# ateme-developers/SVT-AV1-1

Hardware: AMD Instinct MI355X
Metric: 64x64 SAD-search blocks/sec (higher is better)
Workload: dtype u8; 1 GPU; configs[1]: 64x64 full-pel SAD hierarchical ME (centre check + HME L0/L1/L2 + 64x64-area full-pel search of 85 square PUs), 1080p 8-bit, one reference list

## Files before the change

### svt-av1-1_amd/csrc/me_hme.hip

```cpp
#include <hip/hip_runtime.h>
#include <stdint.h>

#include "../../include/svtav1_hip.h"
#include "me_kernels.h"

namespace svthip {

namespace {
#include "me_hme_impl.h"
}

__global__ void __launch_bounds__(256) hme_center_kernel(const uint8_t* __restrict__ pool, HmeJobTable jobs, svthip_me_params P,
                                                         uint32_t list_index, const svthip_sb_origin* __restrict__ sbs, uint32_t n_sb,
                                                         uint32_t n_jobs, const uint32_t* __restrict__ l0_best_mv64, uint32_t l0_mv_stride,
                                                         svthip_fullpel_desc* __restrict__ out_desc,
                                                         int16_t* __restrict__ out_center, int16_t* __restrict__ hme_state)
{
    __shared__ HmeShared sh;
    __shared__ __attribute__((aligned(16))) uint8_t hme_lds[4 * kHmeLdsPerWave];
    const uint32_t sbi = xcd_item(blockIdx.x, n_sb * n_jobs);
    if (sbi >= n_sb * n_jobs) return;
    const uint32_t job = sbi / n_sb, sb_local = sbi - job * n_sb;
    hme_center_sb(pool, jobs.cur[job], jobs.ref[job], P, list_index, sbs[sb_local].x, sbs[sb_local].y, sbi, l0_best_mv64,
                  l0_mv_stride, out_desc, out_center, hme_state, sh, hme_lds);
}

#ifdef SVTHIP_HME_STAMPS
extern "C" int svthip_debug_hme_stamps(void* host, size_t bytes)
{
    return (int)hipMemcpyFromSymbol(host, HIP_SYMBOL(g_hme_stamps), bytes < sizeof(g_hme_stamps) ? bytes : sizeof(g_hme_stamps));
}
extern "C" int svthip_debug_hme_loop_phases(unsigned long long* host8)
{
    return (int)hipMemcpyFromSymbol(host8, HIP_SYMBOL(g_hme_loop_phase), sizeof(g_hme_loop_phase));
}
#endif

}
```

### svt-av1-1_amd/csrc/me_hme_impl.h

```cpp
#pragma once


typedef const __attribute__((address_space(1))) uint32_t gmem_u32;
struct __attribute__((packed, aligned(1))) gmem_u32x4 { uint32_t v[4]; };

__device__ __forceinline__ uint32_t ldu32(const uint8_t* p)
{
    const uintptr_t a = reinterpret_cast<uintptr_t>(p);
    gmem_u32* q = (gmem_u32*)(a & ~(uintptr_t)3);
    const uint32_t sh = (uint32_t)(a & 3u);
    const uint32_t lo = q[0];
    const uint32_t hi = sh ? q[1] : 0u;
    return __builtin_amdgcn_alignbyte(hi, lo, sh);
}

__device__ __forceinline__ uint32_t ldu32_nb(const uint8_t* p)
{
    const uintptr_t a = reinterpret_cast<uintptr_t>(p);
    gmem_u32* q = (gmem_u32*)(a & ~(uintptr_t)3);
    return __builtin_amdgcn_alignbyte(q[1], q[0], (uint32_t)(a & 3u));
}

__device__ __forceinline__ uint32_t wave_sum_u32(uint32_t v)
{
#pragma unroll
    for (int m = 1; m < 64; m <<= 1) v += __shfl_xor(v, m);
    return v;
}

#ifdef SVTHIP_HME_NO_PRIO
#define HME_PRIO(p) do { } while (0)
#else
#define HME_PRIO(p) __builtin_amdgcn_s_setprio(p)
#endif
#ifdef SVTHIP_HME_STAMPS
__device__ unsigned long long g_hme_stamps[8192 * 4 * 8];
#define HME_STAMP(i)                                                                                                          \
    do {                                                                                                                      \
        if (lane == 0 && sbi < 8192u) g_hme_stamps[((size_t)sbi * 4 + (threadIdx.x >> 6)) * 8 + (i)] = __builtin_amdgcn_s_memtime(); \
    } while (0)
__device__ unsigned long long g_hme_loop_phase[2 * 4];
#define HME_LOOP_T(var) const unsigned long long var = __builtin_amdgcn_s_memtime()
#define HME_LOOP_ADD(slot, t1, t0)                                                                                \
    do {                                                                                                          \
        if (lane == 0) atomicAdd(&g_hme_loop_phase[(W == 64 ? 4 : 0) + (slot)], (unsigned long long)((t1) - (t0))); \
    } while (0)
#else
#define HME_STAMP(i) do { } while (0)
#define HME_LOOP_T(var) do { } while (0)
#define HME_LOOP_ADD(slot, t1, t0) do { } while (0)
#endif

__device__ __forceinline__ unsigned long long wave_min_u64(unsigned long long v)
{
#pragma unroll
    for (int m = 1; m < 64; m <<= 1) {
        unsigned long long o = __shfl_xor(v, m);
        v = o < v ? o : v;
    }
    return v;
}

__device__ uint32_t wave_block_sad(const uint8_t* src, uint32_t src_stride, const uint8_t* ref, uint32_t ref_stride,
                                   uint32_t H, uint32_t W, int lane, const uint32_t* src_lds = nullptr)
{
    if (src_lds && W == 64 && H == 32) {
        const uint32_t c = (uint32_t)lane & 15u, r0 = (uint32_t)lane >> 4;
        const uint8_t* rp = ref + (size_t)r0 * ref_stride + 4u * c;
        uint32_t tv[8], acc4 = 0;
#pragma unroll
        for (int k = 0; k < 8; k++) tv[k] = ldu32_nb(rp + (size_t)(4 * k) * ref_stride);
#pragma unroll
        for (int k = 0; k < 8; k++) acc4 = __builtin_amdgcn_sad_u8(src_lds[(r0 + 4 * k) * 16 + c], tv[k], acc4);
        return wave_sum_u32(acc4);
    }
    if (W == 64 && (H & 3u) == 0) {
        const uint32_t c = (uint32_t)lane & 15u, r0 = (uint32_t)lane >> 4;
        const uint8_t* sp = src + (size_t)r0 * src_stride + 4u * c;
        const uint8_t* rp = ref + (size_t)r0 * ref_stride + 4u * c;
        uint32_t acc4 = 0;
        for (uint32_t r = 0; r < H; r += 16) {
            uint32_t sv[4], tv[4];
#pragma unroll
            for (int k = 0; k < 4; k++) {
                const bool in = r + 4u * (uint32_t)k < H;
                sv[k] = in ? *reinterpret_cast<const uint32_t*>(sp + (size_t)(4 * k) * src_stride) : 0u;
                tv[k] = in ? ldu32_nb(rp + (size_t)(4 * k) * ref_stride) : 0u;
            }
#pragma unroll
            for (int k = 0; k < 4; k++) acc4 = __builtin_amdgcn_sad_u8(sv[k], tv[k], acc4);
            sp += (size_t)16 * src_stride;
            rp += (size_t)16 * ref_stride;
        }
        return wave_sum_u32(acc4);
    }
    const uint32_t ndw = (W + 3) >> 2;
    const uint32_t n = H * ndw;
    uint32_t acc = 0;
    for (uint32_t i = lane; i < n; i += 64) {
        const uint32_t r = i / ndw, c = i - r * ndw;
        uint32_t s = ldu32(src + (size_t)r * src_stride + 4 * c);
        uint32_t t = ldu32(ref + (size_t)r * ref_stride + 4 * c);
        const uint32_t rem = W - 4 * c;
        if (rem < 4) {
            const uint32_t m = (1u << (8 * rem)) - 1u;
            s &= m;
            t &= m;
        }
        acc = __builtin_amdgcn_sad_u8(s, t, acc);
    }
    return wave_sum_u32(acc);
}

__device__ void wave_sad_loop_generic(const uint8_t* src, uint32_t src_stride, const uint8_t* ref, uint32_t ref_stride,
                                      uint32_t H, uint32_t W, uint32_t ref_stride_raw, int sw, int sh, int lane,
                                      uint32_t* best_sad, int* bx, int* by)
{
    const int npos = sw * sh;
    unsigned long long best = ~0ull;
    const uint32_t ndw = (W + 3) >> 2;
    const uint32_t tail = W & 3u;
    const uint32_t tailmask = tail ? ((1u << (8 * tail)) - 1u) : 0xffffffffu;
#pragma unroll 1
    for (int pos = lane; pos < npos; pos += 64) {
        const int y = pos / sw, x = pos - y * sw;
        const uint8_t* r0 = ref + (size_t)y * ref_stride_raw + x;
        uint32_t acc = 0;
#pragma unroll 1
        for (uint32_t r = 0; r < H; r++) {
            const uint8_t* sp = src + (size_t)r * src_stride;
            const uint8_t* rp = r0 + (size_t)r * ref_stride;
#pragma unroll 2
            for (uint32_t c = 0; c < ndw; c++) {
                uint32_t s = ldu32(sp + 4 * c);
                uint32_t t = ldu32(rp + 4 * c);
                if (c == ndw - 1) {
                    s &= tailmask;
                    t &= tailmask;
                }
                acc = __builtin_amdgcn_sad_u8(s, t, acc);
            }
        }
        const unsigned long long key = ((unsigned long long)acc << 32) | (uint32_t)pos;
        best = key < best ? key : best;
    }
    best = wave_min_u64(best);
    const uint32_t pos = (uint32_t)__builtin_amdgcn_readfirstlane((int)(uint32_t)best);
    *best_sad = (uint32_t)__builtin_amdgcn_readfirstlane((int)(uint32_t)(best >> 32));
    *by = (int)(pos / (uint32_t)sw);
    *bx = (int)(pos - (uint32_t)(*by) * (uint32_t)sw);
}

__device__ __forceinline__ uint32_t min3u(uint32_t a, uint32_t b, uint32_t c)
{
    uint32_t r;
    asm("v_min3_u32 %0, %1, %2, %3" : "=v"(r) : "v"(a), "v"(b), "v"(c));
    return r;
}

__device__ __forceinline__ uint64_t pack64(uint32_t lo, uint32_t hi) { return ((uint64_t)hi << 32) | lo; }

__device__ __forceinline__ void stage_window_rows(const uint8_t* base, uint32_t ref_stride_raw, int wrows, int pitch, uint32_t* win,
                                                  int lane)
{
    constexpr int NP = 6;
    const int lpr = (pitch + 3) >> 2;
    const int rpp = lpr < 64 ? 64 / lpr : 1;
    const int g = (int)(((uint32_t)lane * ((1u << 16) / (uint32_t)lpr + 1u)) >> 16), q4 = 4 * (lane - g * lpr);
    const bool lane_ok = g < rpp;
    const uintptr_t a0 = reinterpret_cast<uintptr_t>(base) + 4u * (uint32_t)q4;
    for (int r0 = g; r0 < wrows; r0 += NP * rpp) {
        gmem_u32x4 w[NP];
#pragma unroll
        for (int u = 0; u < NP; u++) {
            const int r = min(r0 + u * rpp, wrows - 1);
            const __attribute__((address_space(1))) gmem_u32x4* q = (const __attribute__((address_space(1))) gmem_u32x4*)(a0 + (size_t)r * ref_stride_raw);
#pragma unroll
            for (int k = 0; k < 4; k++) w[u].v[k] = q->v[k];
        }
#pragma unroll
        for (int u = 0; u < NP; u++) {
            const int r = r0 + u * rpp;
            if (lane_ok && r < wrows) {
                uint32_t* o = win + r * pitch + q4;
#pragma unroll
                for (int k = 0; k < 4; k++)
                    if (q4 + k < pitch) o[k] = w[u].v[k];
            }
        }
    }
}

template <int W, bool KEY32 = false>
__device__ void wave_sad_loop_lds(const uint8_t* src, uint32_t src_stride, const uint8_t* ref, uint32_t ref_stride_raw,
                                  int H, int sw, int sh, int lane, uint8_t* lds, int lds_bytes, uint32_t* best_sad,
                                  int* bx, int* by, const uint32_t* shared_src = nullptr)
{
    constexpr int WD = W / 4;
    constexpr int FLUSH = (W == 16) ? 16 : (W == 32 ? 8 : 4);
    const int own_src = shared_src ? 0 : H * WD;
    const uint32_t* srcbuf = shared_src ? shared_src : reinterpret_cast<const uint32_t*>(lds);
    const int noct = (sw + 7) >> 3;
    const int pitch = 2 * noct + WD + 1;
    uint32_t* win = reinterpret_cast<uint32_t*>(lds) + own_src;
    const int avail_rows = (lds_bytes / 4 - own_src) / pitch;
    int band = avail_rows - (2 * H - 2);
    if (band > sh) band = sh;
    if (band < 1) {
        wave_sad_loop_generic(src, src_stride, ref, ref_stride_raw * 2, (uint32_t)H, (uint32_t)W, ref_stride_raw, sw, sh, lane,
                              best_sad, bx, by);
        return;
    }

    for (int i0 = 0; !shared_src && i0 < H * WD; i0 += 256) {
        uint32_t v[4];
#pragma unroll
        for (int k = 0; k < 4; k++) {
            const int i = min(i0 + k * 64 + lane, H * WD - 1);
            const int r = i / WD, c = i - r * WD;
            v[k] = ldu32_nb(src + (uint32_t)r * src_stride + 4u * (uint32_t)c);
        }
#pragma unroll
        for (int k = 0; k < 4; k++) reinterpret_cast<uint32_t*>(lds)[min(i0 + k * 64 + lane, H * WD - 1)] = v[k];
    }

    const int items_row = noct;
    unsigned long long best = ~0ull;
    uint32_t best32 = 0xffffffffu;

    for (int y0 = 0; y0 < sh; y0 += band) {
        const int bh = min(band, sh - y0);
        const int wrows = bh + 2 * H - 2;
        HME_LOOP_T(t_a);
        HME_PRIO(3);
        stage_window_rows(ref + (size_t)y0 * ref_stride_raw, ref_stride_raw, wrows, pitch, win, lane);
        __builtin_amdgcn_wave_barrier();
        asm volatile("s_waitcnt vmcnt(0) lgkmcnt(0)" ::: "memory");
        HME_PRIO(0);
        HME_LOOP_T(t_b);
        HME_LOOP_ADD(0, t_b, t_a);

        const int nitems = items_row * bh;
        int RP = 1, rp_shift = 0;
        while (RP < 8 && nitems * RP * 2 <= 64 && RP * 2 <= H) { RP <<= 1; rp_shift++; }
        const int ipw = 64 >> rp_shift;
        const int part = lane & (RP - 1);
        const uint32_t inv_items = (1u << 20) / (uint32_t)items_row + 1u;
        for (int it0 = 0; it0 < nitems; it0 += ipw) {
            const int item = it0 + (lane >> rp_shift);
            const bool valid = item < nitems;
            const int iy = valid ? (int)(((uint32_t)item * inv_items) >> 20) : 0;
            const int io = valid ? item - iy * items_row : 0;
            uint32_t sad[8];
#pragma unroll
            for (int j = 0; j < 8; j++) sad[j] = 0;
            uint64_t acc0 = 0, acc1 = 0;
            int since = 0;
            for (int r = part; r < H; r += RP) {
                const uint32_t* wr = win + (iy + 2 * r) * pitch + 2 * io;
                const uint32_t* sr = srcbuf + r * WD;
                uint32_t d[WD + 2];
#pragma unroll
                for (int c = 0; c < WD + 2; c++) d[c] = wr[c];
#pragma unroll
                for (int c = 0; c < WD; c++) {
                    const uint32_t sv = sr[c];
                    acc0 = __builtin_amdgcn_qsad_pk_u16_u8(pack64(d[c], d[c + 1]), sv, acc0);
                    acc1 = __builtin_amdgcn_qsad_pk_u16_u8(pack64(d[c + 1], d[c + 2]), sv, acc1);
                }
                if (++since == FLUSH) {
                    since = 0;
                    sad[0] += (uint32_t)acc0 & 0xffffu; sad[1] += ((uint32_t)acc0) >> 16;
                    sad[2] += (uint32_t)(acc0 >> 32) & 0xffffu; sad[3] += (uint32_t)(acc0 >> 48);
                    sad[4] += (uint32_t)acc1 & 0xffffu; sad[5] += ((uint32_t)acc1) >> 16;
                    sad[6] += (uint32_t)(acc1 >> 32) & 0xffffu; sad[7] += (uint32_t)(acc1 >> 48);
                    acc0 = acc1 = 0;
                }
            }
            sad[0] += (uint32_t)acc0 & 0xffffu; sad[1] += ((uint32_t)acc0) >> 16;
            sad[2] += (uint32_t)(acc0 >> 32) & 0xffffu; sad[3] += (uint32_t)(acc0 >> 48);
            sad[4] += (uint32_t)acc1 & 0xffffu; sad[5] += ((uint32_t)acc1) >> 16;
            sad[6] += (uint32_t)(acc1 >> 32) & 0xffffu; sad[7] += (uint32_t)(acc1 >> 48);
            for (int m = 1; m < RP; m <<= 1) {
#pragma unroll
                for (int j = 0; j < 8; j++) sad[j] += __shfl_xor(sad[j], m);
            }
            if (valid && part == 0) {
                const int ys = y0 + iy;
#pragma unroll
                for (int j = 0; j < 8; j++) {
                    const int xs = 8 * io + j;
                    if (xs < sw) {
                        if (KEY32) {
                            best32 = min(best32, (sad[j] << 12) | (uint32_t)(ys * sw + xs));
                        } else {
                            const unsigned long long key = ((unsigned long long)sad[j] << 32) | (uint32_t)(ys * sw + xs);
                            best = key < best ? key : best;
                        }
                    }
                }
            }
        }
        __builtin_amdgcn_wave_barrier();
        HME_LOOP_T(t_c);
        HME_LOOP_ADD(1, t_c, t_b);
    }
    HME_LOOP_T(t_d);
    if (KEY32) {
#pragma unroll
        for (int m = 1; m < 64; m <<= 1) best32 = min(best32, (uint32_t)__shfl_xor((int)best32, m));
        best = ((unsigned long long)(best32 >> 12) << 32) | (best32 & 0xfffu);
    } else {
        best = wave_min_u64(best);
    }
    const uint32_t pos = (uint32_t)__builtin_amdgcn_readfirstlane((int)(uint32_t)best);
    *best_sad = (uint32_t)__builtin_amdgcn_readfirstlane((int)(uint32_t)(best >> 32));
    *by = (int)(pos / (uint32_t)sw);
    *bx = (int)(pos - (uint32_t)(*by) * (uint32_t)sw);
    HME_LOOP_T(t_e);
    HME_LOOP_ADD(2, t_e, t_d);
    HME_LOOP_ADD(3, 1ull, 0ull);
}

__device__ void wave_sad_loop_l0(const uint8_t* src, uint32_t src_stride, const uint8_t* ref, uint32_t ref_stride_raw, int sw, int sh,
                                 int lane, uint8_t* lds, int lds_bytes, uint32_t* best_sad, int* bx, int* by,
                                 const uint32_t* shared_src = nullptr)
{
    constexpr int H = 8, WD = 4;
    const int own_src = shared_src ? 0 : H * WD;
    const uint32_t* srcbuf = shared_src ? shared_src : reinterpret_cast<const uint32_t*>(lds);
    const int nit = (sw + 15) >> 4;
    const int pitch = 4 * nit + 4;
    uint32_t* win = reinterpret_cast<uint32_t*>(lds) + own_src;
    const int avail_rows = (lds_bytes / 4 - own_src) / pitch;
    int band = avail_rows - (2 * H - 2);
    if (band > sh) band = sh;
    if (band < 1 || sw * sh > 65536) {
        wave_sad_loop_lds<16>(src, src_stride, ref, ref_stride_raw, H, sw, sh, lane, lds, lds_bytes, best_sad, bx, by, shared_src);
        return;
    }
    if (!shared_src && lane < H * WD)
        reinterpret_cast<uint32_t*>(lds)[lane] = ldu32_nb(src + (uint32_t)(lane >> 2) * src_stride + 4u * (uint32_t)(lane & 3));
    uint32_t best = 0xffffffffu;
    const uint32_t inv_nit = (1u << 20) / (uint32_t)nit + 1u;
    for (int y0 = 0; y0 < sh; y0 += band) {
        const int bh = min(band, sh - y0);
        HME_PRIO(3);
        stage_window_rows(ref + (size_t)y0 * ref_stride_raw, ref_stride_raw, bh + 2 * H - 2, pitch, win, lane);
        __builtin_amdgcn_wave_barrier();
        asm volatile("s_waitcnt vmcnt(0) lgkmcnt(0)" ::: "memory");
        HME_PRIO(0);
        const int nitems = nit * bh;
        auto track = [&](const uint64_t* acc, int iy, int io, bool valid) {
            const int xs0 = 16 * io;
            const uint32_t base = (uint32_t)((y0 + iy) * sw + xs0);
            if ((sw & 15) == 0) {
                uint32_t lb = 0xffffffffu;
#pragma unroll
                for (int g = 0; g < 4; g++) {
                    const uint32_t lo = (uint32_t)acc[g], hi = (uint32_t)(acc[g] >> 32), ix = base + 4u * (uint32_t)g;
                    lb = min3u((lo << 16) | ix, (lo & 0xffff0000u) | (ix + 1u), lb);
                    lb = min3u((hi << 16) | (ix + 2u), (hi & 0xffff0000u) | (ix + 3u), lb);
                }
                best = min(best, valid ? lb : 0xffffffffu);
                return;
            }
#pragma unroll
            for (int g = 0; g < 4; g++) {
                const uint32_t lo = (uint32_t)acc[g], hi = (uint32_t)(acc[g] >> 32);
                const uint32_t sad4[4] = {lo << 16, lo & 0xffff0000u, hi << 16, hi & 0xffff0000u};
#pragma unroll
                for (int j = 0; j < 4; j++) {
                    const int xs = xs0 + 4 * g + j;
                    const uint32_t key = (valid && xs < sw) ? (sad4[j] + base + (uint32_t)(4 * g + j)) : 0xffffffffu;
                    best = min(best, key);
                }
            }
        };
        auto row_sads = [&](const uint32_t* wr, int r, uint64_t* acc) {
            const uint4 da = *reinterpret_cast<const uint4*>(wr);
            const uint4 db = *reinterpret_cast<const uint4*>(wr + 4);
            const uint4 sv = *reinterpret_cast<const uint4*>(srcbuf + r * WD);
            const uint32_t d[8] = {da.x, da.y, da.z, da.w, db.x, db.y, db.z, db.w};
            const uint32_t s4[4] = {sv.x, sv.y, sv.z, sv.w};
#pragma unroll
            for (int c = 0; c < WD; c++)
#pragma unroll
                for (int g = 0; g < 4; g++)
                    acc[g] = __builtin_amdgcn_qsad_pk_u16_u8(pack64(d[c + g], d[c + g + 1]), s4[c], acc[g]);
        };
        int it0 = 0;
        for (; nitems - it0 >= 57; it0 += 64) {
            const int item = min(it0 + lane, nitems - 1);
            const bool valid = it0 + lane < nitems;
            const int iy = (int)(((uint32_t)item * inv_nit) >> 20), io = item - iy * nit;
            const uint32_t* w0 = win + iy * pitch + 4 * io;
            uint64_t acc[4] = {0, 0, 0, 0};
#pragma unroll
            for (int r = 0; r < H; r++) row_sads(w0 + 2 * r * pitch, r, acc);
            track(acc, iy, io, valid);
        }
        while (it0 < nitems) {
            const int rem = nitems - it0;
            const int rp_shift = rem > 32 ? 1 : rem > 16 ? 1 : rem > 8 ? 2 : 3;
            const int RP = 1 << rp_shift, take = min(rem, 64 >> rp_shift);
            const int slot = lane >> rp_shift, part = lane & (RP - 1);
            const int item = it0 + min(slot, take - 1);
            const int iy = (int)(((uint32_t)item * inv_nit) >> 20), io = item - iy * nit;
            const uint32_t* w0 = win + iy * pitch + 4 * io;
            uint64_t acc[4] = {0, 0, 0, 0};
            for (int r = part; r < H; r += RP) row_sads(w0 + 2 * r * pitch, r, acc);
            for (int m = 1; m < RP; m <<= 1) {
#pragma unroll
                for (int g = 0; g < 4; g++) {
                    const uint32_t lo = (uint32_t)acc[g] + (uint32_t)__shfl_xor((int)(uint32_t)acc[g], m);
                    const uint32_t hi = (uint32_t)(acc[g] >> 32) + (uint32_t)__shfl_xor((int)(uint32_t)(acc[g] >> 32), m);
                    acc[g] = pack64(lo, hi);
                }
            }
            track(acc, iy, io, slot < take && part == 0);
            it0 += take;
        }
        __builtin_amdgcn_wave_barrier();
    }
#pragma unroll
    for (int m = 1; m < 64; m <<= 1) best = min(best, (uint32_t)__shfl_xor((int)best, m));
    best = (uint32_t)__builtin_amdgcn_readfirstlane((int)best);
    const uint32_t pos = best & 0xffffu;
    *best_sad = best >> 16;
    *by = (int)(pos / (uint32_t)sw);
    *bx = (int)(pos - (uint32_t)(*by) * (uint32_t)sw);
}

__device__ __forceinline__ void clamp_center(int& x, int& y, int ox, int oy, int pw, int ph)
{
    x = (ox + x < -63) ? (-63 - ox) : x;
    x = (ox + x > pw - 1) ? (x - ((ox + x) - (pw - 1))) : x;
    y = (oy + y < -63) ? (-63 - oy) : y;
    y = (oy + y > ph - 1) ? (y - ((oy + y) - (ph - 1))) : y;
}

__device__ __forceinline__ void clip_window(int& xo, int& yo, int& sw, int& sh, int ox, int oy, int padw, int padh,
                                            int pw, int ph)
{
    xo = (ox + xo < -padw) ? (-padw - ox) : xo;
    sw = (ox + xo < -padw) ? (sw - (-padw - (ox + xo))) : sw;
    xo = (ox + xo > pw - 1) ? (xo - ((ox + xo) - (pw - 1))) : xo;
    sw = (ox + xo + sw > pw) ? max(1, sw - ((ox + xo + sw) - pw)) : sw;
    yo = (oy + yo < -padh) ? (-padh - oy) : yo;
    sh = (oy + yo < -padh) ? (sh - (-padh - (oy + yo))) : sh;
    yo = (oy + yo > ph - 1) ? (yo - ((oy + yo) - (ph - 1))) : yo;
    sh = (oy + yo + sh > ph) ? max(1, sh - ((oy + yo + sh) - ph)) : sh;
}

__device__ __forceinline__ int s16(int v) { return (int)(int16_t)v; }

__device__ __forceinline__ int round_hme_width(int w)
{
    return (w < 8) ? 8 : ((w & 7) ? (w + (w - ((w >> 3) << 3))) : w);
}

constexpr int kHmeLdsPerWave = 6 * 1024;

struct HmeShared {
    unsigned long long cost[8];
    int rx[3][4], ry[3][4];
    unsigned long long rs[3][4];
    int cx, cy;
    svthip_fullpel_desc desc;
    __attribute__((aligned(16))) uint32_t src2[32 * 16];
    __attribute__((aligned(16))) uint32_t src1[16 * 8];
    __attribute__((aligned(16))) uint32_t src0[8 * 4];
};


__device__ __forceinline__ void hme_center_sb(const uint8_t* __restrict__ pool, const svthip_pa_picture& cur, const svthip_pa_picture& ref,
                                              const svthip_me_params& P, uint32_t list_index, int ox, int oy, uint32_t sbi,
                                              const uint32_t* __restrict__ l0_best_mv64, uint32_t l0_mv_stride,
                                              svthip_fullpel_desc* __restrict__ out_desc, int16_t* __restrict__ out_center,
                                              int16_t* __restrict__ hme_state, HmeShared& sh, uint8_t* hme_lds)
{
    const int tid = threadIdx.x, lane = tid & 63;
    const int wave = __builtin_amdgcn_readfirstlane(tid >> 6);
    uint8_t* wlds = hme_lds + wave * kHmeLdsPerWave;
    const int pw = cur.width, ph = cur.height;
    const uint32_t sb_w = (uint32_t)min(64, pw - ox), sb_h = (uint32_t)min(64, ph - oy);
    const int nw = P.number_hme_search_region_in_width, nh = P.number_hme_search_region_in_height;

    const uint8_t* cur_full = pool + cur.full_offset + (size_t)68 * cur.full_stride + 68;
    const uint8_t* ref_full = pool + ref.full_offset + (size_t)68 * ref.full_stride + 68;
    const uint8_t* src = cur_full + (size_t)oy * cur.full_stride + ox;
    HME_STAMP(0);
    HME_PRIO(3);

    const bool full_sb = sb_w == 64 && sb_h == 64;
    if (full_sb) {
#pragma unroll
        for (int k = 0; k < 2; k++) {
            const int i = tid + 256 * k;
            sh.src2[i] = *reinterpret_cast<const uint32_t*>(src + (size_t)(i >> 4) * (cur.full_stride * 2) + 4 * (i & 15));
        }
        if (tid < 128) {
            const uint8_t* s1 = pool + cur.quarter_offset + (size_t)(32 + (oy >> 1)) * cur.quarter_stride + 32 + (ox >> 1);
            sh.src1[tid] = ldu32_nb(s1 + (size_t)(tid >> 3) * (cur.quarter_stride * 2) + 4 * (tid & 7));
        } else if (tid < 160) {
            const int i = tid - 128;
            const uint8_t* s0 = pool + cur.sixteenth_offset + (size_t)(16 + (oy >> 2)) * cur.sixteenth_stride + 16 + (ox >> 2);
            sh.src0[i] = ldu32_nb(s0 + (size_t)(i >> 2) * (cur.sixteenth_stride * 2) + 4 * (i & 3));
        }
        __syncthreads();
    }
    const uint32_t* src2_lds = full_sb ? sh.src2 : nullptr;
    HME_STAMP(1);

    const bool center_path = (P.temporal_layer_index > 0) || (list_index == 0);
    const uint32_t mv64 = (list_index == 1 && l0_best_mv64) ? l0_best_mv64[(size_t)sbi * l0_mv_stride] : 0u;
    const int dx = s16(0 - (s16((int)(mv64 & 0xffffu)) >> 2));
    const int dy = s16(0 - (s16((int)(mv64 >> 16)) >> 2));
    const int tw = P.hme_level0_total_search_area_width, th = P.hme_level0_total_search_area_height;

    if (tid == 0 && hme_state && list_index == 0) hme_state[25 * (size_t)sbi + 24] = 0;
    int xc = 0, yc = 0;
    if (center_path) {
        int cxs[5] = {0, tw, 0, 0, dx}, cys[5] = {0, 0, -th, th, dy};
        const int ncand = (list_index == 1) ? 5 : 4;
        for (int c = wave; c < ncand; c += 4) {
            int x = cxs[c], y = cys[c];
            clamp_center(x, y, ox, oy, ref.width, ref.height);
            const uint32_t sad = wave_block_sad(src, cur.full_stride * 2, ref_full + (size_t)(oy + y) * ref.full_stride + ox + x,
                                                ref.full_stride * 2, sb_h >> 1, sb_w, lane, src2_lds);
            if (lane == 0) sh.cost[c] = (unsigned long long)(sad << 1) << 8;
        }
        __syncthreads();
        {
            const unsigned long long zero = sh.cost[0], b = sh.cost[1], c = sh.cost[2], d = sh.cost[3];
            const unsigned long long dir = (list_index == 1) ? sh.cost[4] : 0xFFFFFFFFFFFFFull;
            unsigned long long best = zero;
            best = b < best ? b : best;
            best = c < best ? c : best;
            best = d < best ? d : best;
            best = dir < best ? dir : best;
            if (best == zero) { xc = 0; yc = 0; }
            else if (best == b) { xc = tw; yc = 0; }
            else if (best == c) { xc = 0; yc = s16(0 - th); }
            else if (best == dir) { xc = dx; yc = dy; }
            else { xc = 0; yc = th; }
        }

        if (P.enable_hme_flag && sb_h == 64) {
            const int nreg = nw * nh;
            const int16_t* st = hme_state ? hme_state + 25 * (size_t)sbi : nullptr;
            const bool carried = st && list_index == 1 && st[24];
            if (wave < nreg) {
                const int rw = wave % nw, rh = wave / nw;
                const int k = rw * 2 + rh;
                int x0 = xc, y0 = yc, x1 = xc, y1 = yc, x2 = xc, y2 = yc;
                if (carried) { x0 = st[k]; y0 = st[4 + k]; x1 = st[8 + k]; y1 = st[12 + k]; x2 = st[16 + k]; y2 = st[20 + k]; }
                uint32_t sad0 = 0, sad1 = 0, sad2 = 0;
                HME_STAMP(2);
                if (P.enable_hme_level0_flag) {
                    const uint32_t mx = P.hme_level0_multiplier_x, my = P.hme_level0_multiplier_y;
                    int sw = s16((int)((P.hme_level0_search_area_in_width_array[rw] * mx) / 100));
                    int shh = s16((int)((P.hme_level0_search_area_in_height_array[rh] * my) / 100));
                    int xd = s16(xc >> 2), yd = s16(yc >> 2);
                    for (int j = rw; j > 0;) { j--; xd = s16(xd + s16((int)((P.hme_level0_search_area_in_width_array[j] * mx) / 100))); }
                    for (int j = rh; j > 0;) { j--; yd = s16(yd + s16((int)((P.hme_level0_search_area_in_height_array[j] * my) / 100))); }
                    int xo = s16(-s16((int)(((tw * mx) / 100) >> 1)) + xd);
                    int yo = s16(-s16((int)(((th * my) / 100) >> 1)) + yd);
                    const int o_x = ox >> 2, o_y = oy >> 2;
                    clip_window(xo, yo, sw, shh, o_x, o_y, 15, 15, ref.width >> 2, ref.height >> 2);
                    const uint8_t* s = pool + cur.sixteenth_offset + (size_t)(16 + o_y) * cur.sixteenth_stride + 16 + o_x;
                    const uint8_t* r = pool + ref.sixteenth_offset + (size_t)(16 + o_y + yo) * ref.sixteenth_stride + 16 + o_x + xo;
                    int bx, by;
                    if (sb_w == 64)
                        wave_sad_loop_l0(s, cur.sixteenth_stride * 2, r, ref.sixteenth_stride, sw, shh, lane, wlds, kHmeLdsPerWave, &sad0,
                                         &bx, &by, sh.src0);
                    else
                        wave_sad_loop_generic(s, cur.sixteenth_stride * 2, r, ref.sixteenth_stride * 2, (sb_h >> 2) >> 1, sb_w >> 2,
                                              ref.sixteenth_stride, sw, shh, lane, &sad0, &bx, &by);
                    x0 = s16(s16(bx + xo) * 4);
                    y0 = s16(s16(by + yo) * 4);
                }
                HME_STAMP(3);
                if (P.enable_hme_level1_flag) {
                    int sw = round_hme_width((int)(int16_t)P.hme_level1_search_area_in_width_array[rw]);
                    int shh = (int)(int16_t)P.hme_level1_search_area_in_height_array[rh];
                    int xo = s16(-(sw >> 1) + (x0 >> 1)), yo = s16(-(shh >> 1) + (y0 >> 1));
                    const int o_x = ox >> 1, o_y = oy >> 1;
                    clip_window(xo, yo, sw, shh, o_x, o_y, 31, 31, ref.width >> 1, ref.height >> 1);
                    const uint8_t* s = pool + cur.quarter_offset + (size_t)(32 + o_y) * cur.quarter_stride + 32 + o_x;
                    const uint8_t* r = pool + ref.quarter_offset + (size_t)(32 + o_y + yo) * ref.quarter_stride + 32 + o_x + xo;
                    int bx, by;
                    if (sb_w == 64 && sw * shh <= 4096)
                        wave_sad_loop_lds<32, true>(s, cur.quarter_stride * 2, r, ref.quarter_stride, 16, sw, shh, lane, wlds,
                                                    kHmeLdsPerWave, &sad1, &bx, &by, sh.src1);
                    else if (sb_w == 64)
                        wave_sad_loop_lds<32>(s, cur.quarter_stride * 2, r, ref.quarter_stride, 16, sw, shh, lane, wlds,
                                              kHmeLdsPerWave, &sad1, &bx, &by, sh.src1);
                    else
                        wave_sad_loop_generic(s, cur.quarter_stride * 2, r, ref.quarter_stride * 2, (sb_h >> 1) >> 1, sb_w >> 1,
                                              ref.quarter_stride, sw, shh, lane, &sad1, &bx, &by);
                    x1 = s16(s16(bx + xo) * 2);
                    y1 = s16(s16(by + yo) * 2);
                }
                HME_STAMP(4);
                if (P.enable_hme_level2_flag) {
                    int sw = round_hme_width((int)(int16_t)P.hme_level2_search_area_in_width_array[rw]);
                    int shh = (int)(int16_t)P.hme_level2_search_area_in_height_array[rh];
                    int xo = s16(-(sw >> 1) + x1), yo = s16(-(shh >> 1) + y1);
                    clip_window(xo, yo, sw, shh, ox, oy, 63, 63, ref.width, ref.height);
                    const uint8_t* r = ref_full + (size_t)(oy + yo) * ref.full_stride + ox + xo;
                    int bx, by;
                    if (sb_w == 64 && sw * shh <= 4096)
                        wave_sad_loop_lds<64, true>(src, cur.full_stride * 2, r, ref.full_stride, 32, sw, shh, lane, wlds,
                                                    kHmeLdsPerWave, &sad2, &bx, &by, sh.src2);
                    else if (sb_w == 64)
                        wave_sad_loop_lds<64>(src, cur.full_stride * 2, r, ref.full_stride, 32, sw, shh, lane, wlds,
                                              kHmeLdsPerWave, &sad2, &bx, &by, sh.src2);
                    else
                        wave_sad_loop_generic(src, cur.full_stride * 2, r, ref.full_stride * 2, sb_h >> 1, sb_w, ref.full_stride, sw,
                                              shh, lane, &sad2, &bx, &by);
                    x2 = s16(bx + xo);
                    y2 = s16(by + yo);
                }
                HME_STAMP(5);
                if (lane == 0) {
                    sh.rx[0][k] = x0; sh.ry[0][k] = y0; sh.rs[0][k] = (unsigned long long)sad0 * 2;
                    sh.rx[1][k] = x1; sh.ry[1][k] = y1; sh.rs[1][k] = (unsigned long long)sad1 * 2;
                    sh.rx[2][k] = x2; sh.ry[2][k] = y2; sh.rs[2][k] = (unsigned long long)sad2 * 2;
                }
            }
            __syncthreads();
            if (tid == 0) {
                int lvl = -1;
                if (P.enable_hme_level0_flag && !P.enable_hme_level1_flag && !P.enable_hme_level2_flag) lvl = 0;
                if (P.enable_hme_level1_flag && !P.enable_hme_level2_flag) lvl = 1;
                if (P.enable_hme_level2_flag) lvl = 2;
                int xh = 0, yh = 0;
                if (lvl >= 0) {
                    xh = sh.rx[lvl][0]; yh = sh.ry[lvl][0];
                    unsigned long long bs = sh.rs[lvl][0];
                    int w = 1, h = 0;
                    while (h < nh) {
                        while (w < nw) {
                            const int k = w * 2 + h;
                            if (sh.rs[lvl][k] < bs) { xh = sh.rx[lvl][k]; yh = sh.ry[lvl][k]; bs = sh.rs[lvl][k]; }
                            w++;
                        }
                        w = 0;
                        h++;
                    }
                }
                if (P.enable_hme_level2_flag) {
                    const int total = nh * nw;
                    if (P.ref_poc_equal && list_index == 1 && total > 1) {
                        for (int q = 0; q < total - 1; q++)
                            for (int n = q + 1; n < total; n++) {
                                const int a = (q / nw) * 2 + (q % nw), b = (n / nw) * 2 + (n % nw);
                                if (sh.rs[2][a] > sh.rs[2][b]) {
                                    const int tx = sh.rx[2][a], ty = sh.ry[2][a];
                                    const unsigned long long ts = sh.rs[2][a];
                                    sh.rx[2][a] = sh.rx[2][b]; sh.ry[2][a] = sh.ry[2][b]; sh.rs[2][a] = sh.rs[2][b];
                                    sh.rx[2][b] = tx; sh.ry[2][b] = ty; sh.rs[2][b] = ts;
                                }
                            }
                        xh = sh.rx[2][1];
                        yh = sh.ry[2][1];
                    }
                }
                sh.cx = xh;
                sh.cy = yh;
                if (hme_state) {
                    int16_t* so = hme_state + 25 * (size_t)sbi;
                    for (int k = 0; k < 4; k++) {
                        const bool live = ((k >> 1) < nw) && ((k & 1) < nh);
                        for (int l = 0; l < 3; l++) {
                            so[8 * l + k] = (int16_t)(live ? sh.rx[l][k] : (carried ? so[8 * l + k] : 0));
                            so[8 * l + 4 + k] = (int16_t)(live ? sh.ry[l][k] : (carried ? so[8 * l + 4 + k] : 0));
                        }
                    }
                    so[24] = 1;
                }
            }
            __syncthreads();
            xc = sh.cx;
            yc = sh.cy;
        }
    }

    HME_PRIO(3);
    if ((xc != 0 || yc != 0) && P.is_used_as_reference_flag) {
        clamp_center(xc, yc, ox, oy, ref.width, ref.height);
        __syncthreads();
        if (wave < 2) {
            const int x = wave ? xc : 0, y = wave ? yc : 0;
            const uint32_t sad = wave_block_sad(src, cur.full_stride * 2, ref_full + (size_t)(oy + y) * ref.full_stride + ox + x,
                                                ref.full_stride * 2, sb_h >> 1, sb_w, lane, src2_lds);
            if (lane == 0) sh.cost[6 + wave] = (unsigned long long)(sad << 1) << 8;
        }
        __syncthreads();
        const unsigned long long z = sh.cost[6], hcost = sh.cost[7];
        const unsigned long long m = z < hcost ? z : hcost;
        if (m == z) { xc = 0; yc = 0; }
    }

    HME_STAMP(6);
    if (tid == 0) {
        int sw = min((int)P.search_area_width, 127), shh = min((int)P.search_area_height, 127);
        int xo = s16(xc - (sw >> 1)), yo = s16(yc - (shh >> 1));
        clip_window(xo, yo, sw, shh, ox, oy, 63, 63, pw, ph);
        svthip_fullpel_desc d;
        d.src_offset = (int32_t)(cur.full_offset + (int64_t)(68 + oy) * cur.full_stride + 68 + ox);
        d.ref_offset = (int32_t)(ref.full_offset + (int64_t)(68 + oy + yo) * ref.full_stride + 68 + ox + xo);
        d.x_search_area_origin = xo;
        d.y_search_area_origin = yo;
        d.search_area_width = sw;
        d.search_area_height = shh;
        out_desc[sbi] = d;
        sh.desc = d;
        if (out_center) {
            out_center[2 * sbi] = (int16_t)xc;
            out_center[2 * sbi + 1] = (int16_t)yc;
        }
    }
}
```

Baseline: 9.110 million blocks/s.

## Prefetch HME centre candidates, add fixed-size QSAD loops, reuse level-2 cost

Before the source is staged into LDS, each wave now loads the reference rows for its own centre candidate, so that load latency overlaps the staging. It also adds compile-time specialised QSAD search loops for the common 16x16 quarter-res and 8x8 full-res window sizes, using DPP reductions and packed 32-bit keys. It tracks which level-2 result is selected and reuses its SAD and the zero-MV centre cost, skipping the final re-evaluation of both blocks and two barriers when that is valid. The per-wave LDS slice grows to 7KB, which may reduce occupancy. The cost-reuse bookkeeping also adds a risk of subtle mismatches in which centre is chosen.

```diff
diff --git a/svt-av1-1_amd/csrc/me_hme.hip b/svt-av1-1_amd/csrc/me_hme.hip
--- a/svt-av1-1_amd/csrc/me_hme.hip
+++ b/svt-av1-1_amd/csrc/me_hme.hip
@@ -3,6 +3,7 @@
 
 #include "../../include/svtav1_hip.h"
 #include "me_kernels.h"
+#include "me_wave_reduce.h"
 
 namespace svthip {
 
diff --git a/svt-av1-1_amd/csrc/me_hme_impl.h b/svt-av1-1_amd/csrc/me_hme_impl.h
--- a/svt-av1-1_amd/csrc/me_hme_impl.h
+++ b/svt-av1-1_amd/csrc/me_hme_impl.h
@@ -51,6 +51,8 @@
 #define HME_LOOP_ADD(slot, t1, t0) do { } while (0)
 #endif
 
+constexpr int kHmeLdsPerWave = 7 * 1024;
+
 __device__ __forceinline__ unsigned long long wave_min_u64(unsigned long long v)
 {
 #pragma unroll
@@ -61,18 +63,30 @@
     return v;
 }
 
+__device__ __forceinline__ void load_ref_block64(const uint8_t* ref, uint32_t ref_stride, int lane, uint32_t (&tv)[8])
+{
+    const uint32_t c = (uint32_t)lane & 15u, r0 = (uint32_t)lane >> 4;
+    const uint8_t* rp = ref + (size_t)r0 * ref_stride + 4u * c;
+#pragma unroll
+    for (int k = 0; k < 8; k++) tv[k] = ldu32_nb(rp + (size_t)(4 * k) * ref_stride);
+}
+
+__device__ __forceinline__ uint32_t sad_ref_block64(const uint32_t (&tv)[8], const uint32_t* src_lds, int lane)
+{
+    const uint32_t c = (uint32_t)lane & 15u, r0 = (uint32_t)lane >> 4;
+    uint32_t acc4 = 0;
+#pragma unroll
+    for (int k = 0; k < 8; k++) acc4 = __builtin_amdgcn_sad_u8(src_lds[(r0 + 4 * k) * 16 + c], tv[k], acc4);
+    return wave_sum_u32(acc4);
+}
+
 __device__ uint32_t wave_block_sad(const uint8_t* src, uint32_t src_stride, const uint8_t* ref, uint32_t ref_stride,
                                    uint32_t H, uint32_t W, int lane, const uint32_t* src_lds = nullptr)
 {
     if (src_lds && W == 64 && H == 32) {
-        const uint32_t c = (uint32_t)lane & 15u, r0 = (uint32_t)lane >> 4;
-        const uint8_t* rp = ref + (size_t)r0 * ref_stride + 4u * c;
-        uint32_t tv[8], acc4 = 0;
-#pragma unroll
-        for (int k = 0; k < 8; k++) tv[k] = ldu32_nb(rp + (size_t)(4 * k) * ref_stride);
-#pragma unroll
-        for (int k = 0; k < 8; k++) acc4 = __builtin_amdgcn_sad_u8(src_lds[(r0 + 4 * k) * 16 + c], tv[k], acc4);
-        return wave_sum_u32(acc4);
+        uint32_t tv[8];
+        load_ref_block64(ref, ref_stride, lane, tv);
+        return sad_ref_block64(tv, src_lds, lane);
     }
     if (W == 64 && (H & 3u) == 0) {
         const uint32_t c = (uint32_t)lane & 15u, r0 = (uint32_t)lane >> 4;
@@ -322,6 +336,100 @@
     HME_LOOP_ADD(3, 1ull, 0ull);
 }
 
+template <int W, int H, int SW, int SH>
+__device__ void wave_sad_loop_fixed(const uint8_t* ref, uint32_t ref_stride_raw, int lane, uint8_t* lds, const uint32_t* srcbuf,
+                                    uint32_t* best_sad, int* bx, int* by)
+{
+    constexpr int WD = W / 4;
+    constexpr int NQ = SW / 4;
+    constexpr int RP = 64 / SH;
+    constexpr int ROWS = H / RP;
+    constexpr int ND = WD + NQ;
+    constexpr int PITCH = (ND + 3) & ~3;
+    constexpr int WROWS = SH + 2 * H - 2;
+    static_assert(RP * SH == 64 && ROWS * RP == H && (RP & (RP - 1)) == 0 && RP >= 2 && RP <= 8, "one wave pass, RP a power of two");
+    static_assert(ROWS * W * 255 < 65536 && H * W * 255 < (1 << 20) && SW * SH <= 4096 && (SW & (SW - 1)) == 0, "u16 sums, 32-bit keys");
+    static_assert(WROWS * PITCH * 4 <= kHmeLdsPerWave, "the window fits the slice");
+    typedef __attribute__((address_space(3))) uint32_t lds_u32;
+    typedef uint32_t u32x4_t __attribute__((ext_vector_type(4)));
+    typedef uint32_t u32x2_t __attribute__((ext_vector_type(2)));
+
+    uint32_t* win = reinterpret_cast<uint32_t*>(lds);
+    HME_PRIO(3);
+    stage_window_rows(ref, ref_stride_raw, WROWS, PITCH, win, lane);
+    __builtin_amdgcn_wave_barrier();
+    asm volatile("s_waitcnt vmcnt(0) lgkmcnt(0)" ::: "memory");
+    HME_PRIO(0);
+
+    const int iy = lane / RP, part = lane & (RP - 1);
+    const uint32_t* w0 = win + (iy + 2 * part) * PITCH;
+    uint64_t acc[NQ];
+#pragma unroll
+    for (int g = 0; g < NQ; g++) acc[g] = 0;
+#pragma unroll
+    for (int i = 0; i < ROWS; i++) {
+        const int r = part + RP * i;
+        const uint32_t* wr = w0 + 2 * RP * i * PITCH;
+        lds_u32* wo = (lds_u32*)wr;
+        asm("" : "+v"(wo));
+        uint32_t d[PITCH];
+#pragma unroll
+        for (int k = 0; k < PITCH / 4; k++) {
+            if (4 * k + 2 >= ND) {
+                u32x2_t v = *reinterpret_cast<const u32x2_t*>(wr + 4 * k);
+                asm("" : "+v"(v));
+                d[4 * k] = v.x; d[4 * k + 1] = v.y; d[4 * k + 2] = d[4 * k + 3] = 0;
+            } else {
+                u32x4_t v = *reinterpret_cast<const u32x4_t*>(wr + 4 * k);
+                asm("" : "+v"(v));
+                d[4 * k] = v.x; d[4 * k + 1] = v.y; d[4 * k + 2] = v.z; d[4 * k + 3] = v.w;
+            }
+        }
+        uint64_t odd[ND / 2];
+#pragma unroll
+        for (int k = 1; k + 1 < ND; k += 2) odd[k / 2] = pack64(wo[k], wo[k + 1]);
+        uint32_t sv[WD];
+#pragma unroll
+        for (int k = 0; k < WD / 4; k++) {
+            const uint4 v = *reinterpret_cast<const uint4*>(srcbuf + r * WD + 4 * k);
+            sv[4 * k] = v.x; sv[4 * k + 1] = v.y; sv[4 * k + 2] = v.z; sv[4 * k + 3] = v.w;
+        }
+#pragma unroll
+        for (int c = 0; c < WD; c++)
+#pragma unroll
+            for (int g = 0; g < NQ; g++) {
+                const int k = c + g;
+                acc[g] = __builtin_amdgcn_qsad_pk_u16_u8((k & 1) ? odd[k / 2] : pack64(d[k], d[k + 1]), sv[c], acc[g]);
+            }
+    }
+    __builtin_amdgcn_wave_barrier();
+
+    uint32_t key = 0xffffffffu;
+#pragma unroll
+    for (int g = 0; g < NQ; g++) {
+        uint32_t v[4] = {(uint32_t)acc[g] & 0xffffu, (uint32_t)acc[g] >> 16, (uint32_t)(acc[g] >> 32) & 0xffffu, (uint32_t)(acc[g] >> 48)};
+#pragma unroll
+        for (int j = 0; j < 4; j++) {
+            v[j] += dpp_fetch<0xB1>(v[j]);
+            v[j] += dpp_fetch<0x4E>(v[j]);
+            if (RP == 8) v[j] += dpp_fetch<0x141>(v[j]);
+        }
+        key = min3u((v[0] << 12) | (uint32_t)(4 * g), (v[1] << 12) | (uint32_t)(4 * g + 1), key);
+        key = min3u((v[2] << 12) | (uint32_t)(4 * g + 2), (v[3] << 12) | (uint32_t)(4 * g + 3), key);
+    }
+    key |= (uint32_t)(iy * SW);
+    key = min(key, dpp_fetch<0xB1>(key));
+    key = min(key, dpp_fetch<0x4E>(key));
+    key = min(key, dpp_fetch<0x124>(key));
+    key = min(key, dpp_fetch<0x128>(key));
+    const uint32_t best = min(min((uint32_t)__builtin_amdgcn_readlane((int)key, 0), (uint32_t)__builtin_amdgcn_readlane((int)key, 16)),
+                              min((uint32_t)__builtin_amdgcn_readlane((int)key, 32), (uint32_t)__builtin_amdgcn_readlane((int)key, 48)));
+    const uint32_t pos = best & 0xfffu;
+    *best_sad = best >> 12;
+    *by = (int)(pos / (uint32_t)SW);
+    *bx = (int)(pos % (uint32_t)SW);
+}
+
 __device__ void wave_sad_loop_l0(const uint8_t* src, uint32_t src_stride, const uint8_t* ref, uint32_t ref_stride_raw, int sw, int sh,
                                  int lane, uint8_t* lds, int lds_bytes, uint32_t* best_sad, int* bx, int* by,
                                  const uint32_t* shared_src = nullptr)
@@ -460,13 +568,12 @@
     return (w < 8) ? 8 : ((w & 7) ? (w + (w - ((w >> 3) << 3))) : w);
 }
 
-constexpr int kHmeLdsPerWave = 6 * 1024;
-
 struct HmeShared {
     unsigned long long cost[8];
     int rx[3][4], ry[3][4];
     unsigned long long rs[3][4];
     int cx, cy;
+    unsigned long long hcost;
     svthip_fullpel_desc desc;
     __attribute__((aligned(16))) uint32_t src2[32 * 16];
     __attribute__((aligned(16))) uint32_t src1[16 * 8];
@@ -493,7 +600,15 @@
     HME_STAMP(0);
     HME_PRIO(3);
 
+    const bool center_path = (P.temporal_layer_index > 0) || (list_index == 0);
+    const int tw = P.hme_level0_total_search_area_width, th = P.hme_level0_total_search_area_height;
     const bool full_sb = sb_w == 64 && sb_h == 64;
+    uint32_t cand_tv[8];
+    if (full_sb && center_path) {
+        int x = wave == 1 ? tw : 0, y = wave == 2 ? -th : (wave == 3 ? th : 0);
+        clamp_center(x, y, ox, oy, ref.width, ref.height);
+        load_ref_block64(ref_full + (size_t)(oy + y) * ref.full_stride + ox + x, ref.full_stride * 2, lane, cand_tv);
+    }
     if (full_sb) {
 #pragma unroll
         for (int k = 0; k < 2; k++) {
@@ -513,22 +628,26 @@
     const uint32_t* src2_lds = full_sb ? sh.src2 : nullptr;
     HME_STAMP(1);
 
-    const bool center_path = (P.temporal_layer_index > 0) || (list_index == 0);
     const uint32_t mv64 = (list_index == 1 && l0_best_mv64) ? l0_best_mv64[(size_t)sbi * l0_mv_stride] : 0u;
     const int dx = s16(0 - (s16((int)(mv64 & 0xffffu)) >> 2));
     const int dy = s16(0 - (s16((int)(mv64 >> 16)) >> 2));
-    const int tw = P.hme_level0_total_search_area_width, th = P.hme_level0_total_search_area_height;
 
     if (tid == 0 && hme_state && list_index == 0) hme_state[25 * (size_t)sbi + 24] = 0;
     int xc = 0, yc = 0;
+    unsigned long long hme_cost = ~0ull;
     if (center_path) {
-        int cxs[5] = {0, tw, 0, 0, dx}, cys[5] = {0, 0, -th, th, dy};
         const int ncand = (list_index == 1) ? 5 : 4;
+        const int cxs[5] = {0, tw, 0, 0, dx}, cys[5] = {0, 0, -th, th, dy};
         for (int c = wave; c < ncand; c += 4) {
-            int x = cxs[c], y = cys[c];
-            clamp_center(x, y, ox, oy, ref.width, ref.height);
-            const uint32_t sad = wave_block_sad(src, cur.full_stride * 2, ref_full + (size_t)(oy + y) * ref.full_stride + ox + x,
-                                                ref.full_stride * 2, sb_h >> 1, sb_w, lane, src2_lds);
+            uint32_t sad;
+            if (full_sb && c == wave) {
+                sad = sad_ref_block64(cand_tv, src2_lds, lane);
+            } else {
+                int x = cxs[c], y = cys[c];
+                clamp_center(x, y, ox, oy, ref.width, ref.height);
+                sad = wave_block_sad(src, cur.full_stride * 2, ref_full + (size_t)(oy + y) * ref.full_stride + ox + x, ref.full_stride * 2,
+                                     sb_h >> 1, sb_w, lane, src2_lds);
+            }
             if (lane == 0) sh.cost[c] = (unsigned long long)(sad << 1) << 8;
         }
         __syncthreads();
@@ -591,7 +710,9 @@
                     const uint8_t* s = pool + cur.quarter_offset + (size_t)(32 + o_y) * cur.quarter_stride + 32 + o_x;
                     const uint8_t* r = pool + ref.quarter_offset + (size_t)(32 + o_y + yo) * ref.quarter_stride + 32 + o_x + xo;
                     int bx, by;
-                    if (sb_w == 64 && sw * shh <= 4096)
+                    if (sb_w == 64 && sw == 16 && shh == 16)
+                        wave_sad_loop_fixed<32, 16, 16, 16>(r, ref.quarter_stride, lane, wlds, sh.src1, &sad1, &bx, &by);
+                    else if (sb_w == 64 && sw * shh <= 4096)
                         wave_sad_loop_lds<32, true>(s, cur.quarter_stride * 2, r, ref.quarter_stride, 16, sw, shh, lane, wlds,
                                                     kHmeLdsPerWave, &sad1, &bx, &by, sh.src1);
                     else if (sb_w == 64)
@@ -611,7 +732,9 @@
                     clip_window(xo, yo, sw, shh, ox, oy, 63, 63, ref.width, ref.height);
                     const uint8_t* r = ref_full + (size_t)(oy + yo) * ref.full_stride + ox + xo;
                     int bx, by;
-                    if (sb_w == 64 && sw * shh <= 4096)
+                    if (sb_w == 64 && sw == 8 && shh == 8)
+                        wave_sad_loop_fixed<64, 32, 8, 8>(r, ref.full_stride, lane, wlds, sh.src2, &sad2, &bx, &by);
+                    else if (sb_w == 64 && sw * shh <= 4096)
                         wave_sad_loop_lds<64, true>(src, cur.full_stride * 2, r, ref.full_stride, 32, sw, shh, lane, wlds,
                                                     kHmeLdsPerWave, &sad2, &bx, &by, sh.src2);
                     else if (sb_w == 64)
@@ -637,9 +760,10 @@
                 if (P.enable_hme_level1_flag && !P.enable_hme_level2_flag) lvl = 1;
                 if (P.enable_hme_level2_flag) lvl = 2;
                 int xh = 0, yh = 0;
+                unsigned long long bs = ~0ull;
                 if (lvl >= 0) {
                     xh = sh.rx[lvl][0]; yh = sh.ry[lvl][0];
-                    unsigned long long bs = sh.rs[lvl][0];
+                    bs = sh.rs[lvl][0];
                     int w = 1, h = 0;
                     while (h < nh) {
                         while (w < nw) {
@@ -651,25 +775,33 @@
                         h++;
                     }
                 }
+                unsigned long long hcost = lvl == 2 ? bs << 8 : ~0ull;
                 if (P.enable_hme_level2_flag) {
                     const int total = nh * nw;
                     if (P.ref_poc_equal && list_index == 1 && total > 1) {
+                        uint32_t from = 0xE4u;
                         for (int q = 0; q < total - 1; q++)
                             for (int n = q + 1; n < total; n++) {
                                 const int a = (q / nw) * 2 + (q % nw), b = (n / nw) * 2 + (n % nw);
                                 if (sh.rs[2][a] > sh.rs[2][b]) {
                                     const int tx = sh.rx[2][a], ty = sh.ry[2][a];
+                                    const uint32_t fa = (from >> (2 * a)) & 3u, fb = (from >> (2 * b)) & 3u;
                                     const unsigned long long ts = sh.rs[2][a];
                                     sh.rx[2][a] = sh.rx[2][b]; sh.ry[2][a] = sh.ry[2][b]; sh.rs[2][a] = sh.rs[2][b];
                                     sh.rx[2][b] = tx; sh.ry[2][b] = ty; sh.rs[2][b] = ts;
+                                    from ^= ((fa ^ fb) << (2 * a)) | ((fa ^ fb) << (2 * b));
                                 }
                             }
                         xh = sh.rx[2][1];
                         yh = sh.ry[2][1];
+                        const uint32_t f1 = (from >> 2) & 3u;
+                        const bool live = (int)(f1 >> 1) < nw && (int)(f1 & 1u) < nh;
+                        hcost = live ? sh.rs[2][1] << 8 : ~0ull;
                     }
                 }
                 sh.cx = xh;
                 sh.cy = yh;
+                sh.hcost = hcost;
                 if (hme_state) {
                     int16_t* so = hme_state + 25 * (size_t)sbi;
                     for (int k = 0; k < 4; k++) {
@@ -685,21 +817,29 @@
             __syncthreads();
             xc = sh.cx;
             yc = sh.cy;
+            hme_cost = sh.hcost;
         }
     }
 
     HME_PRIO(3);
     if ((xc != 0 || yc != 0) && P.is_used_as_reference_flag) {
         clamp_center(xc, yc, ox, oy, ref.width, ref.height);
-        __syncthreads();
-        if (wave < 2) {
-            const int x = wave ? xc : 0, y = wave ? yc : 0;
-            const uint32_t sad = wave_block_sad(src, cur.full_stride * 2, ref_full + (size_t)(oy + y) * ref.full_stride + ox + x,
-                                                ref.full_stride * 2, sb_h >> 1, sb_w, lane, src2_lds);
-            if (lane == 0) sh.cost[6 + wave] = (unsigned long long)(sad << 1) << 8;
-        }
-        __syncthreads();
-        const unsigned long long z = sh.cost[6], hcost = sh.cost[7];
+        unsigned long long z, hcost;
+        if (hme_cost != ~0ull && ox < ref.width && oy < ref.height) {
+            z = sh.cost[0];
+            hcost = hme_cost;
+        } else {
+            __syncthreads();
+            if (wave < 2) {
+                const int x = wave ? xc : 0, y = wave ? yc : 0;
+                const uint32_t sad = wave_block_sad(src, cur.full_stride * 2, ref_full + (size_t)(oy + y) * ref.full_stride + ox + x,
+                                                    ref.full_stride * 2, sb_h >> 1, sb_w, lane, src2_lds);
+                if (lane == 0) sh.cost[6 + wave] = (unsigned long long)(sad << 1) << 8;
+            }
+            __syncthreads();
+            z = sh.cost[6];
+            hcost = sh.cost[7];
+        }
         const unsigned long long m = z < hcost ? z : hcost;
         if (m == z) { xc = 0; yc = 0; }
     }
```

Measured after the change: 9.553 million blocks/s, median of 6. +4.9%, better.
